# nianticlabs/relpose-gnn

Measured on AMD Instinct MI355X. Metric: graphs/sec (8-node fully-connected, 224x224), higher is better.
Workload: dtype f32; 1 GPU; BASELINE.json configs[1]: batch=32 8-node fully-connected graphs per GPU, 224x224 RGB, fp32, ResNet34 + GNN (D=2048, gnn_recursion=2, droprate=0, eval), random-init weights; nodes_per_graph=8, edges_per_graph=56, streams_per_gpu=2, loaded_library=relpose-gnn_amd/lib/librelpose_gnn_hip.so@b255fe2efddb

## Files before the change

relpose-gnn_amd/csrc/gemm_f32.hip:

```cpp
#include <atomic>
#include <map>
#include <mutex>
#include <type_traits>
#include <utility>
#include <vector>

#include "rpg_common.h"

typedef float f32x16 __attribute__((ext_vector_type(16)));

namespace {


struct Epilogue {
    const float* scale;
    const float* shift;
    const float* residual;
    float* out;
    int ldc;
    int relu;
    const int64_t* res_idx = nullptr;
    const float* residual2 = nullptr;
    const int64_t* res2_idx = nullptr;
    int ldr = 0;
// ... 520 lines not shown
    const long span = 256 / ((long)ho * wo) + 2;
    int seg = span * h * wd * cin * 4 >= (1L << 31) ? 0 : (cin % 32 == 0 ? 32 : (cin % 16 == 0 ? 16 : 0));
    if (cin == 4 && kh * kw <= 64 && kw >= 4 && span * h * wd * cin * 4 < (1L << 31)) seg = -1;
    launch_tiles<ConvKind, ConvArgs>(a, w, (int)K, (int)M, cout, (int)K, ep, s, seg);
    timing_end(slot, 2.0 * (double)M * cout * (double)kh * kw * (alg_cin > 0 ? alg_cin : cin), s, t_executed);
    RPG_CHECK_LAUNCH("conv2d_bn_act");
    return RPG_OK;
}

int launch_linear(const GatherSrc& src, const float* weight, const float* bias, const float* residual, float* out,
                  int m, int n_out, int relu, hipStream_t s, const GatherRes* gres, float* out_relu) {
    if (src.n < 1 || src.n > 3 || !weight || !out || m <= 0 || n_out <= 0 || !aligned16(weight)) return RPG_ERR_BAD_ARG;
    GatherArgs a{};
    int K = 0;
    for (int i = 0; i < 3; ++i) {
        if (i < src.n) {
            if (!src.a[i] || src.width[i] <= 0 || (src.width[i] & 3) || (src.ld[i] & 3) || src.ld[i] < src.width[i] ||
                !aligned16(src.a[i]))
                return RPG_ERR_BAD_ARG;
            a.a[i] = src.a[i]; a.idx[i] = src.idx[i]; a.ld[i] = src.ld[i];
            K += src.width[i];
        } else {
            a.a[i] = nullptr; a.idx[i] = nullptr; a.ld[i] = 0;
        }
    }
    a.w0 = src.width[0];
    a.w01 = src.n >= 2 ? src.width[0] + src.width[1] : K;
    a.K = K;
    a.fold_k = g_fold_k;
    Epilogue ep{nullptr, bias, residual, out, n_out, relu};
    ep.out_relu = out_relu;
    if (out_relu && !aligned16(out_relu)) return RPG_ERR_BAD_ARG;
    if (gres) {
        if (!gres->res1 || !gres->idx1 || gres->ld < n_out || (gres->res2 && !gres->idx2)) return RPG_ERR_BAD_ARG;
        ep.residual = gres->res1; ep.res_idx = gres->idx1;
        ep.residual2 = gres->res2; ep.res2_idx = gres->idx2;
        ep.ldr = gres->ld;
    }
    const int slot = timing_begin(RPG_TIMER_LINEAR, s);
    int seg = 32;
    for (int i = 0; i < src.n; ++i) {
        if (src.width[i] % 32) seg = src.width[i] % 16 ? 0 : (seg ? 16 : 0);
        const long rows = src.idx[i] ? src.rows[i] : (long)m;
        if (rows <= 0 || rows * src.ld[i] * 4 >= (1L << 31)) seg = 0;
    }
    if (!(src.n == 1 && !src.idx[0] && launch_linear112(src.a[0], src.ld[0], weight, K, m, n_out, K, ep, s)))
        launch_tiles<GatherKind, GatherArgs>(a, weight, K, m, n_out, K, ep, s, seg);
    timing_end(slot, 2.0 * (double)m * n_out * (double)K, s, t_executed);
    RPG_CHECK_LAUNCH("linear_gather");
    return RPG_OK;
}

}

extern "C" int rpg_conv2d_bn_act_nhwc_f32(const float* x, const float* w_ohwi, const float* scale, const float* shift,
                                          const float* residual, float* y, int n, int h, int w, int cin, int cout,
                                          int kh, int kw, int stride, int pad, int relu, void* stream) {
    return rpg::launch_conv(x, w_ohwi, scale, shift, residual, y, n, h, w, cin, cout, kh, kw, stride, pad, relu,
                            rpg::as_stream(stream));
}

extern "C" int rpg_linear_gather_f32(int n_src, const float* const* a, const int64_t* const* idx, const int* ld,
                                     const int* width, const float* weight, const float* bias, const float* residual,
                                     float* out, int m, int n_out, int relu, void* stream) {
    if (n_src < 1 || n_src > 3 || !a || !ld || !width) return RPG_ERR_BAD_ARG;
    rpg::GatherSrc src{};
    src.n = n_src;
    for (int i = 0; i < n_src; ++i) {
        src.a[i] = a[i];
        src.idx[i] = idx ? idx[i] : nullptr;
        src.ld[i] = ld[i];
        src.width[i] = width[i];
    }
    return rpg::launch_linear(src, weight, bias, residual, out, m, n_out, relu, rpg::as_stream(stream));
}

extern "C" int rpg_linear_gather_ex_f32(int n_src, const float* const* a, const int64_t* const* idx, const int* ld,
                                        const int* width, const long* rows, const float* weight, const float* bias,
                                        const float* residual, const int64_t* res_idx, const float* residual2,
                                        const int64_t* res2_idx, int ldr, float* out, float* out_relu, int m, int n_out,
                                        int relu, void* stream) {
    if (n_src < 1 || n_src > 3 || !a || !ld || !width) return RPG_ERR_BAD_ARG;
    rpg::GatherSrc src{};
    src.n = n_src;
    for (int i = 0; i < n_src; ++i) {
        src.a[i] = a[i];
        src.idx[i] = idx ? idx[i] : nullptr;
        src.ld[i] = ld[i];
        src.width[i] = width[i];
        src.rows[i] = rows ? rows[i] : 0;
    }
    if (!res_idx && !residual2)
        return (res2_idx || (residual && ldr && ldr != n_out)) ? RPG_ERR_BAD_ARG
               : rpg::launch_linear(src, weight, bias, residual, out, m, n_out, relu, rpg::as_stream(stream), nullptr, out_relu);
    rpg::GatherRes gr{residual, res_idx, residual2, res2_idx, ldr};
    return rpg::launch_linear(src, weight, bias, nullptr, out, m, n_out, relu, rpg::as_stream(stream), &gr, out_relu);
}

extern "C" int rpg_release_scratch(void) {
    if (hipDeviceSynchronize() != hipSuccess) {
        rpg::set_last_error("release_scratch", hipGetLastError());
        return RPG_ERR_LAUNCH;
    }
    std::lock_guard<std::mutex> lk(g_scratch_mu);
    for (auto& kv : g_scratch)
        if (kv.second.p) (void)hipFree(kv.second.p);
    g_scratch.clear();
    for (float* p : g_retired) (void)hipFree(p);
    g_retired.clear();
    return RPG_OK;
}

extern "C" int rpg_set_tuning(int key, int value) {
    switch (key) {
        case RPG_TUNE_FIXUP_PRIO: g_fixup_prio = value != 0; return RPG_OK;
        case RPG_TUNE_BF16_PAIR: rpg::bf16_set_pair(value != 0); return RPG_OK;
        case RPG_TUNE_TILE: g_force_tile = value; return RPG_OK;
        case RPG_TUNE_BK: if (value != 0 && value != 16 && value != 32) return RPG_ERR_BAD_ARG; g_bk = value; return RPG_OK;
        case RPG_TUNE_EPILOGUE: g_epi_lds = value != 0; return RPG_OK;
        case RPG_TUNE_STREAMK: g_streamk = value != 0; return RPG_OK;
        case RPG_TUNE_BF16_BK: if (value != 32 && value != 64) return RPG_ERR_BAD_ARG; rpg::bf16_set_bk(value); return RPG_OK;
        case RPG_TUNE_INKERNEL_FIXUP:
            if (value < 0 || value > 7) return RPG_ERR_BAD_ARG;
            g_inkernel_fixup = value & 3;
            rpg::wino_combine_max_set((value & 4) ? 32 : 8);
            return RPG_OK;
        case RPG_TUNE_GNN_SPLIT: g_gnn_split = value != 0; return RPG_OK;
        case RPG_TUNE_GNN_FUSE_AGG: g_gnn_fuse_agg = value != 0; return RPG_OK;
        case RPG_TUNE_LIN112: if (value < 0 || value > 3) return RPG_ERR_BAD_ARG; g_lin112 = value; return RPG_OK;
        case RPG_TUNE_FOLD_K: if (value < 0 || (value % 64)) return RPG_ERR_BAD_ARG; g_fold_k = value; return RPG_OK;
        case RPG_TUNE_FAST_LOADER: g_fast = value != 0; return RPG_OK;
        case RPG_TUNE_WAVES8: g_waves8 = value != 0; return RPG_OK;
        case RPG_TUNE_WINO_SPLIT: if (value < 0 || value > 96) return RPG_ERR_BAD_ARG; rpg::wino_split_set(value); return RPG_OK;
        case RPG_TUNE_BF16_TILE: if (value < -1 || value > 3) return RPG_ERR_BAD_ARG; rpg::bf16_set_tile(value); return RPG_OK;
        case RPG_TUNE_BF16_FAST: rpg::bf16_set_fast(value != 0); return RPG_OK;
        case RPG_TUNE_BF16_LEAN_EPI: rpg::bf16_set_lean_epi(value != 0); return RPG_OK;
        case RPG_TUNE_BF16_PERSIST: rpg::bf16_set_persist(value != 0); return RPG_OK;
        case RPG_TUNE_BF16_FUSE_BLOCK: rpg::bf16_set_fuse_block((int)(value & 7)); return RPG_OK;
        case RPG_TUNE_BF16_TAIL: if (value < 0 || value > 7) return RPG_ERR_BAD_ARG; rpg::bf16_set_tail(value); return RPG_OK;
        case RPG_TUNE_BF16_LINEAR_DMA: if (value != 0 && (value < 10 || value > 19)) return RPG_ERR_BAD_ARG; rpg::bf16_set_linear_dma(value); return RPG_OK;
        case RPG_TUNE_WINO2D:
            if (value < 0 || value > 2 || (value != 0 && rpg_wino43_weights_floats(1, 1) != 42)) return RPG_ERR_BAD_ARG;
            rpg::wino2d_set(value);
            return RPG_OK;
        case RPG_TUNE_BF16_CHUNK:
            if (value < 0) return RPG_ERR_BAD_ARG;
            rpg::bf16_set_chunk(value & 4095, (value >> 12) ? (value >> 12) : 64);
            return RPG_OK;
        case RPG_TUNE_BF16_PATCH: if (value < 0 || value % 10 > 4 || value > 14) return RPG_ERR_BAD_ARG; rpg::bf16_set_patch(value); return RPG_OK;
        case RPG_TUNE_BF16_DMA: if (value < 0 || value > 40) return RPG_ERR_BAD_ARG; rpg::bf16_set_dma(value); return RPG_OK;
        case RPG_TUNE_SK_MIN_ITS: if (value < 1 || value > 4096) return RPG_ERR_BAD_ARG; SK_MIN_ITS = value; return RPG_OK;
        case RPG_TUNE_BF16_WS64: if (value < 0 || value > 2) return RPG_ERR_BAD_ARG; return rpg::bf16_set_ws64(value);
        case RPG_TUNE_FUSED_STEM: rpg::stem_pool_set((value & 1) != 0); rpg::stem_pool_set_strip((value & 128) != 0, value >> 8); rpg::bf16_set_fused_stem((value & 1) != 0); rpg::bf16_set_stem_strip((value & 2) ? 0 : ((value & 32) ? 1 : 9), value >> 8); return RPG_OK;
        case RPG_TUNE_WINOGRAD: if (value < 0 || (value > 3 && value < 16)) return RPG_ERR_BAD_ARG; rpg::wino_set(value); return RPG_OK;
        case RPG_TUNE_WINO_PERSIST: if (value < 0 || value > 2) return RPG_ERR_BAD_ARG; rpg::wino_persist_set(value); return RPG_OK;
        case RPG_TUNE_WINO_SHORT: if (value < 0) return RPG_ERR_BAD_ARG; rpg::wino_short_set(value); return RPG_OK;
        default: return RPG_ERR_BAD_ARG;
    }
}
```

relpose-gnn_amd/csrc/winograd.hip:

```cpp
#include "rpg_common.h"

typedef float f32x16 __attribute__((ext_vector_type(16)));

namespace {

constexpr int NT = 256;
constexpr int BK = 16, LD = BK;
constexpr int P = 6;
constexpr int BMT = 64, BN = 64;
constexpr int A_FLOATS = P * BMT * LD, B_FLOATS = P * BN * LD;
constexpr int LDS_BYTES = (A_FLOATS + B_FLOATS) * (int)sizeof(float);

struct Epi {
    const float* scale;
    const float* shift;
    const float* residual;
    float* out;
    int relu;
};

__device__ __forceinline__ float4 f4zero() { return make_float4(0.f, 0.f, 0.f, 0.f); }
__device__ __forceinline__ float4 lin(float a, const float4& x, float b, const float4& y) {
    return make_float4(a * x.x + b * y.x, a * x.y + b * y.y, a * x.z + b * y.z, a * x.w + b * y.w);
}
// ... 776 lines not shown
                decode();
            }
        }
    };

    const int st_a = row * LD + 4 * (slot ^ ((row >> 2) & 3));
    const int st_b = A8_FLOATS + (3 * bhalf) * BN * LD + brow * LD + 4 * (slot ^ ((brow >> 2) & 3));
    struct Img { int a[2], b[2], sa, sb; };
    float4* lds4 = reinterpret_cast<float4*>(lds);
    auto stage_one = [&](int p, const Img& I) {
        if (p >= P) {
            lds4[I.sb + (p - P) * (BN * LD / 4)] = ub[p - P];
            return;
        }
#ifdef RPG_ABL_NOXF
        lds4[I.sa + p * (BMT8 * LD / 4)] = d[p];
        return;
#endif
        const F4 d0 = to_f4(d[0]), d1 = to_f4(d[1]), d2 = to_f4(d[2]), d3 = to_f4(d[3]), d4 = to_f4(d[4]), d5 = to_f4(d[5]);
        F4 v;
        if (p == 0) v = fma4_p4(sub4(d0, d2), sub4(d4, d2));
        else if (p == 5) v = fma4_m4(sub4(d3, d1), sub4(d5, d3));
        else if (p <= 2) {
            const F4 sx = fma4_m4(d2, d4);
            const F4 tx = fma4_m4(d1, d3);
            v = p == 1 ? add4(sx, tx) : sub4(sx, tx);
        } else {
            const F4 r = sub4(d4, d2), t = sub4(d3, d1);
            v = p == 3 ? fma4_p2(t, r) : fma4_m2(t, r);
        }
        lds4[I.sa + p * (BMT8 * LD / 4)] = to_float4(v);
    };

    f32x16 acc[P];
    const int rsw = 4 * ((lane >> 5) ^ ((lane >> 2) & 3));
    const int a_off = (wm * 32 + (lane & 31)) * LD + rsw;
    const int b_off = A8_FLOATS + (wn * 32 + (lane & 31)) * LD + rsw;
    float4 fa[2][2], fb[2][2];
    constexpr int IMG4 = IMG8_FLOATS / 4;
    Img X{{a_off >> 2, (a_off ^ 8) >> 2}, {b_off >> 2, (b_off ^ 8) >> 2}, st_a >> 2, st_b >> 2};
    Img Y{{X.a[0] + IMG4, X.a[1] + IMG4}, {X.b[0] + IMG4, X.b[1] + IMG4}, X.sa + IMG4, X.sb + IMG4};
    int ybase = IMG8_FLOATS;
    auto frag_one = [&](int g, int set, int i, const Img& I) {
        const int xi = 2 * (g % 3) + (i >> 1);
        if (i & 1) fb[set][i >> 1] = lds4[I.b[g / 3] + xi * (BN * LD / 4)];
        else       fa[set][i >> 1] = lds4[I.a[g / 3] + xi * (BMT8 * LD / 4)];
    };
    auto kstep = [&](const Img& cur, const Img& nxt, int khf) {
        __builtin_amdgcn_sched_barrier(0);
#pragma unroll
        for (int g = 0; g < 6; ++g) {
            const int set = g & 1, x0 = 2 * (g % 3);
#pragma unroll
            for (int i = 0; i < 8; ++i) {
                const int j = i & 1, e = i >> 1;
                const float av = e == 0 ? fa[set][j].x : e == 1 ? fa[set][j].y : e == 2 ? fa[set][j].z : fa[set][j].w;
                const float bv = e == 0 ? fb[set][j].x : e == 1 ? fb[set][j].y : e == 2 ? fb[set][j].z : fb[set][j].w;
                acc[x0 + j] = __builtin_amdgcn_mfma_f32_32x32x2f32(av, bv, acc[x0 + j], 0, 0, 0);
                if (i < 4) {
                    if (g < 5) frag_one(g + 1, set ^ 1, i, cur);
                    else frag_one(0, 0, i, nxt);
                } else {
                    const int s = 4 * (g % 3) + (i - 4);
                    if (s < 9) {
                        if (g < 3) stage_one(s, nxt);
                        else fetch_one(s, khf);
                    }
                }
                __builtin_amdgcn_sched_barrier(0);
            }
#ifndef RPG_ABL_NOBAR
            if (g == 4) {
                __syncthreads();
                __builtin_amdgcn_sched_barrier(0);
            }
#endif
        }
        fetch_next(khf);
    };

    int c_item = f_item, c_m0 = f_m0, c_n0 = f_n0, c_ns = f_nk - f_kb;
#pragma unroll
    for (int i = 0; i < 9; ++i) fetch_one(i, 0);
    fetch_next(0);
#pragma unroll
    for (int p = 0; p < 9; ++p) stage_one(p, X);
#pragma unroll
    for (int i = 0; i < 9; ++i) fetch_one(i, 1);
    fetch_next(1);
    const int ws = __builtin_amdgcn_readfirstlane(wave);
    for (;;) {
#ifdef RPG_WINO_TRACE
        if (g_wino_trace && threadIdx.x == 0) {
            g_wino_trace[5 * c_item] = __builtin_amdgcn_s_getreg(0xF804);
            g_wino_trace[5 * c_item + 1] = __builtin_readcyclecounter();
        }
#endif
#pragma unroll
        for (int xi = 0; xi < P; ++xi)
#pragma unroll
            for (int e = 0; e < 16; ++e) acc[xi][e] = 0.f;
        __syncthreads();
#pragma unroll
        for (int i = 0; i < 4; ++i) frag_one(0, 0, i, X);
#ifdef RPG_WINO_TRACE
        if (g_wino_trace && threadIdx.x == 0) g_wino_trace[5 * c_item + 2] = __builtin_readcyclecounter();
#endif
        int s = 0;
        for (; s + 6 <= c_ns; s += 6) {
            kstep(X, Y, 2);
            kstep(Y, X, 0);
            kstep(X, Y, 1);
            kstep(Y, X, 2);
            kstep(X, Y, 0);
            kstep(Y, X, 1);
        }
        if (s < c_ns) {
            kstep(X, Y, 2);
            kstep(Y, X, 0);
            kstep(X, Y, 1);
            const Img t = X;
            X = Y;
            Y = t;
            ybase = IMG8_FLOATS - ybase;
        }
        __syncthreads();
        float* slab = lds + ybase + ws * (64 * 36);
#ifdef RPG_WINO_TRACE
        if (g_wino_trace && threadIdx.x == 0) g_wino_trace[5 * c_item + 3] = __builtin_readcyclecounter();
#endif
        auto refetch = [&]() {
            fix_row1();
#pragma unroll
            for (int i = 0; i < 9; ++i) fetch_one(i, 1);
        };
        int lane_e = lane;
        asm volatile("" : "+v"(lane_e));
        if (c_item < sp.n_split)
            wino43_epilogue_partial(acc, slab, lane_e, (ws >> 1) * 32, (ws & 1) * 32,
                                    sp.partial + (size_t)c_item * (BMT8 * 4 * BN), refetch);
        else
            wino43_epilogue_lean(acc, slab, lane_e, c_m0 + (ws >> 1) * 32, c_n0 + (ws & 1) * 32, M, Tw, W, Cout, ep, refetch);
#ifdef RPG_WINO_TRACE
        if (g_wino_trace && threadIdx.x == 0) g_wino_trace[5 * c_item + 4] = __builtin_readcyclecounter();
#endif
        if (f_item >= n_items) break;
        c_item = f_item;
        c_m0 = f_m0;
        c_n0 = f_n0;
        c_ns = f_nk - f_kb;
    }
}

__global__ __launch_bounds__(256) void wino43_fixup_kernel(const float* __restrict__ partial, Epi ep, int M, int Tw, int W,
                                                           int Cout, int tiles_n, Split sp) {
    const int tt = blockIdx.x >> 5, idx = (blockIdx.x & 31) * 256 + threadIdx.x;
    const float* src = partial + (size_t)tt * sp.parts * (BMT8 * 4 * BN) + 4 * idx;
    float4 s = *reinterpret_cast<const float4*>(src);
    for (int i = 1; i < sp.parts; ++i) {
        const float4 v = *reinterpret_cast<const float4*>(src + (size_t)i * (BMT8 * 4 * BN));
        s.x += v.x; s.y += v.y; s.z += v.z; s.w += v.w;
    }
    wino43_finish_quad(s, ep, sp.tile_base + tt, idx >> 4, idx & 15, M, Tw, W, Cout, tiles_n);
}

__global__ __launch_bounds__(NT) void wino43_weights_kernel(const float* __restrict__ w, float* __restrict__ U, int Cout,
                                                            int Cin, long total) {
    const long i = (long)blockIdx.x * NT + threadIdx.x;
    if (i >= total) return;
    const int c = (int)(i % Cin);
    const long t = i / Cin;
    const int kh = (int)(t % 3);
    const long co = t / 3;
    const float* wp = w + ((co * 3 + kh) * 3) * (long)Cin + c;
    const double g0 = wp[0], g1 = wp[Cin], g2 = wp[2 * (long)Cin];
    const double u[6] = {g0 / 4.0, -(g0 + g1 + g2) / 6.0, -(g0 - g1 + g2) / 6.0,
                         g0 / 24.0 + g1 / 12.0 + g2 / 6.0, g0 / 24.0 - g1 / 12.0 + g2 / 6.0, g2};
    const long plane = (long)Cout * 3 * Cin;
#pragma unroll
    for (int xi = 0; xi < 6; ++xi) U[xi * plane + i] = (float)u[xi];
}

int g_wino_split = 1;
int g_wino_split_steps = 3;
int g_wino = 1;
int g_wino_min_blocks = 16;
int g_wino_persist = 1;
int g_wino_combine_max = 8;

}

#ifdef RPG_PROBE_WINO2D
#include "../../tools/probes/winograd2d.hip"
#endif

namespace rpg {

#ifndef RPG_PROBE_WINO2D
void wino2d_set(int) {}
#endif
bool wino_enabled() { return g_wino != 0; }
void wino_set(int on) { if (on >= 16) { g_wino = 1; g_wino_min_blocks = on; } else { g_wino = on; g_wino_min_blocks = 16; } }
void wino_split_set(int v) { g_wino_split = v != 0; g_wino_split_steps = v >= 2 ? v : 3; }
void wino_short_set(int) {}
void wino_persist_set(int on) { g_wino_persist = on; }
void wino_combine_max_set(int v) { g_wino_combine_max = v; }

bool wino_pays(int n, int h, int w, int cin, int cout) {
    if (!g_wino || (cin & 3) || (cout & 3)) return false;
    const long tiles = (long)n * h * ((w + 3) / 4);
    const long blocks = ((tiles + BMT - 1) / BMT) * ((cout + BN - 1) / BN);
    const int tw = (w + 3) / 4;
    return blocks >= g_wino_min_blocks && (long)h * w * cin * 4 * 67 < (1L << 31) && 6L * cout * 3 * cin * 4 < (1L << 31) &&
           (32L / tw + 3) * w * cout * 4 < (1L << 31);
}

int launch_conv_wino(const float* x, const float* u, const float* scale, const float* shift, const float* residual,
                     float* y, int n, int h, int w, int cin, int cout, int relu, hipStream_t s) {
    if (!x || !u || !y || n <= 0 || h <= 0 || w <= 0 || cin <= 0 || cout <= 0 || (cin & 3) || (cout & 3) ||
        !aligned16(x) || !aligned16(u) || !aligned16(y) || (scale && !aligned16(scale)) || (shift && !aligned16(shift)) ||
        (residual && !aligned16(residual)))
        return RPG_ERR_BAD_ARG;
#ifdef RPG_PROBE_WINO2D
    if (wino2d_takes(n, h, w, cin, cout))
        return launch_conv_wino2d(x, u + (size_t)18 * cout * cin, scale, shift, residual, y, n, h, w, cin, cout, relu, s);
#endif
    const int tw = (w + 3) / 4;
    const long M = (long)n * h * tw;
    if (M >= (1L << 31) || (long)h * w * cin * 4 * 67 >= (1L << 31) || 6L * cout * 3 * cin * 4 >= (1L << 31) ||
        (32L / tw + 3) * w * cout * 4 >= (1L << 31))
        return RPG_ERR_BAD_ARG;
    int dev = 0;
    if (hipGetDevice(&dev) != hipSuccess || dev < 0 || dev >= 64) dev = 0;
    static bool attr[64] = {};
    if (!attr[dev]) {
        (void)hipFuncSetAttribute(reinterpret_cast<const void*>(wino43_conv_kernel),
                                  hipFuncAttributeMaxDynamicSharedMemorySize, LDS_BYTES);
        attr[dev] = true;
    }
    const int tn = (cout + BN - 1) / BN;
    Epi ep{scale, shift, residual, y, relu};
    const int slot = timing_begin(RPG_TIMER_CONV_WINO, s);
    double executed = 0.0;
    const long tm8 = (M + BMT8 - 1) / BMT8;
    const bool fits8 = (long)h * w * cin * 4 * 131 < (1L << 31);
    if (fits8 && (g_wino == 3 || (g_wino == 1 && tm8 * tn >= 8))) {
        static bool attr8[64] = {};
        if (!attr8[dev]) {
            (void)hipFuncSetAttribute(reinterpret_cast<const void*>(wino43_conv8_kernel),
                                      hipFuncAttributeMaxDynamicSharedMemorySize, LDS8_BYTES);
            attr8[dev] = true;
        }
        const long T = tm8 * tn;
        const int S = num_cus(), kpr = (cin + BK - 1) / BK, nk = 3 * kpr;
        executed = (double)T * nk * 48.0 * 8.0 * 4096.0;
        long t_main = T;
        Split sp{0, 1, 0, nullptr, nullptr};
        const long tail = T % S;
        if (g_wino_persist && cin % BK == 0 && (T > S || g_wino_persist == 2) && h >= 2) {
            static bool attr8p[64] = {};
            if (!attr8p[dev]) {
                (void)hipFuncSetAttribute(reinterpret_cast<const void*>(wino43_conv8p_kernel),
                                          hipFuncAttributeMaxDynamicSharedMemorySize, LDS8_BYTES);
                attr8p[dev] = true;
            }
            if (g_wino_split && tail > 0) {
                int parts = (int)(S / tail);
                if (parts > kpr) parts = kpr;
                if (parts >= 2) {
                    sp.partial = stream_scratch(s, (size_t)tail * parts * (BMT8 * 4 * BN) * sizeof(float));
                    if (sp.partial) { sp.parts = parts; t_main = T - tail; sp.tile_base = (int)t_main; sp.n_split = (int)(tail * parts); }
                }
            }
            const long items = sp.n_split + t_main;
            hipLaunchKernelGGL(wino43_conv8p_kernel, dim3((unsigned)(items < S ? items : S)), dim3(NT8), LDS8_BYTES, s, x, u, h, w,
                               cin, cout, tw, (int)M, ep, tn, sp, (int)items);
            if (sp.n_split) {
                hipStream_t fs = fixup_hop_begin(s);
                hipLaunchKernelGGL(wino43_fixup_kernel, dim3((unsigned)(T - t_main) * 32), dim3(256), 0, fs, sp.partial, ep, (int)M,
                                   tw, w, cout, tn, sp);
                fixup_hop_end(s, fs);
            }
            timing_end(slot, 2.0 * (double)n * h * w * cout * 9.0 * cin, s, executed);
            RPG_CHECK_LAUNCH("conv3x3_wino43");
            return RPG_OK;
        }
        if (g_wino_split && tail > 0) {
            int parts = (int)(S / tail);
            if (parts > kpr) parts = kpr;
            if (parts > nk / g_wino_split_steps && nk / g_wino_split_steps >= 2) parts = nk / g_wino_split_steps;
            if (parts >= 2) {
                unsigned* counters = nullptr;
                sp.partial = stream_scratch(s, (size_t)tail * parts * (BMT8 * 4 * BN) * sizeof(float), &counters);
                if (sp.partial) { sp.parts = parts; t_main = T - tail; sp.tile_base = (int)t_main; sp.n_split = (int)(tail * parts); }
                if (sp.partial && inkernel_fixup_enabled() && parts <= g_wino_combine_max) sp.arrive = counters;
            }
        }
        hipLaunchKernelGGL(wino43_conv8_kernel, dim3((unsigned)(sp.n_split + t_main)), dim3(NT8), LDS8_BYTES, s, x, u, h, w, cin,
                           cout, tw, (int)M, ep, tn, sp);
        if (sp.n_split && !sp.arrive) {
            hipStream_t fs = fixup_hop_begin(s);
            hipLaunchKernelGGL(wino43_fixup_kernel, dim3((unsigned)(T - t_main) * 32), dim3(256), 0, fs, sp.partial, ep, (int)M, tw, w,
                               cout, tn, sp);
            fixup_hop_end(s, fs);
        }
    } else {
        const int tm = (int)((M + BMT - 1) / BMT);
        executed = (double)tm * tn * (3 * ((cin + BK - 1) / BK)) * 48.0 * 4.0 * 4096.0;
        hipLaunchKernelGGL(wino43_conv_kernel, dim3(tm * tn), dim3(NT), LDS_BYTES, s, x, u, h, w, cin, cout, tw, (int)M, ep, tn);
    }
    timing_end(slot, 2.0 * (double)n * h * w * cout * 9.0 * cin, s, executed);
    RPG_CHECK_LAUNCH("conv3x3_wino43");
    return RPG_OK;
}

}

#ifdef RPG_WINO_TRACE
extern "C" int rpg_wino_trace_set(unsigned long long* buf) {
    return hipMemcpyToSymbol(HIP_SYMBOL(g_wino_trace), &buf, sizeof(buf)) == hipSuccess ? RPG_OK : RPG_ERR_LAUNCH;
}
#endif

extern "C" size_t rpg_wino43_weights_floats(int cout, int cin) {
    if (cout <= 0 || cin <= 0) return 0;
#ifdef RPG_PROBE_WINO2D
    return rpg::wino_weight_floats(cout, cin);
#else
    return (size_t)18 * cout * cin;
#endif
}

extern "C" int rpg_wino43_transform_weights_f32(const float* w_ohwi, float* u, int cout, int cin, void* stream) {
    if (!w_ohwi || !u || cout <= 0 || cin <= 0) return RPG_ERR_BAD_ARG;
    const long total = (long)cout * 3 * cin;
    hipLaunchKernelGGL(wino43_weights_kernel, dim3((unsigned)((total + NT - 1) / NT)), dim3(NT), 0, rpg::as_stream(stream),
                       w_ohwi, u, cout, cin, total);
    RPG_CHECK_LAUNCH("wino43_transform_weights");
#ifdef RPG_PROBE_WINO2D
    return rpg::launch_wino2d_weights(w_ohwi, u + (size_t)18 * cout * cin, cout, cin, rpg::as_stream(stream));
#else
    return RPG_OK;
#endif
}

extern "C" int rpg_conv3x3_wino43_bn_act_nhwc_f32(const float* x, const float* u, const float* scale, const float* shift,
                                                  const float* residual, float* y, int n, int h, int w, int cin, int cout,
                                                  int relu, void* stream) {
    return rpg::launch_conv_wino(x, u, scale, shift, residual, y, n, h, w, cin, cout, relu, rpg::as_stream(stream));
}
```

Measured before the change: 3089 graphs/s.

## Add shared-row Winograd conv kernel reusing input rows across the three kernel rows

Adds a new Winograd F(4,3) conv kernel that stages one transformed input strip plus halo rows in LDS. The kh=0,1,2 kernel-row passes then read shifted windows of the same strip instead of refetching and retransforming input per kernel row. It is enabled by default when the tile width fits, for both the persistent and one-shot launch paths, with a new tune value to disable it. The kernel uses more LDS per block, which may lower occupancy, and adds complex index and halo logic.

```diff
diff --git a/relpose-gnn_amd/csrc/gemm_f32.hip b/relpose-gnn_amd/csrc/gemm_f32.hip
--- a/relpose-gnn_amd/csrc/gemm_f32.hip
+++ b/relpose-gnn_amd/csrc/gemm_f32.hip
@@ -696,7 +696,7 @@
         case RPG_TUNE_SK_MIN_ITS: if (value < 1 || value > 4096) return RPG_ERR_BAD_ARG; SK_MIN_ITS = value; return RPG_OK;
         case RPG_TUNE_BF16_WS64: if (value < 0 || value > 2) return RPG_ERR_BAD_ARG; return rpg::bf16_set_ws64(value);
         case RPG_TUNE_FUSED_STEM: rpg::stem_pool_set((value & 1) != 0); rpg::stem_pool_set_strip((value & 128) != 0, value >> 8); rpg::bf16_set_fused_stem((value & 1) != 0); rpg::bf16_set_stem_strip((value & 2) ? 0 : ((value & 32) ? 1 : 9), value >> 8); return RPG_OK;
-        case RPG_TUNE_WINOGRAD: if (value < 0 || (value > 3 && value < 16)) return RPG_ERR_BAD_ARG; rpg::wino_set(value); return RPG_OK;
+        case RPG_TUNE_WINOGRAD: if (value < 0 || (value > 4 && value < 16)) return RPG_ERR_BAD_ARG; rpg::wino_set(value); return RPG_OK;
         case RPG_TUNE_WINO_PERSIST: if (value < 0 || value > 2) return RPG_ERR_BAD_ARG; rpg::wino_persist_set(value); return RPG_OK;
         case RPG_TUNE_WINO_SHORT: if (value < 0) return RPG_ERR_BAD_ARG; rpg::wino_short_set(value); return RPG_OK;
         default: return RPG_ERR_BAD_ARG;
diff --git a/relpose-gnn_amd/csrc/winograd.hip b/relpose-gnn_amd/csrc/winograd.hip
--- a/relpose-gnn_amd/csrc/winograd.hip
+++ b/relpose-gnn_amd/csrc/winograd.hip
@@ -952,6 +952,343 @@
     }
 }
 
+constexpr int SROWS = 148, SZROW = SROWS - 4;
+constexpr int WINO_SHARED_MAX_TW = (SZROW - BMT8) / 2;
+constexpr int SPLANE = SROWS * LD, SA_FLOATS = P * SPLANE;
+constexpr int S_A0 = 0, S_B0 = SA_FLOATS, S_B1 = S_B0 + B_FLOATS, S_A1 = S_B1 + B_FLOATS;
+constexpr int LDS8S_BYTES = (2 * SA_FLOATS + 2 * B_FLOATS) * (int)sizeof(float);
+static_assert(SA_FLOATS + B_FLOATS >= 8 * 64 * 36, "the epilogue slabs fit in one (A, B) pair");
+static_assert(S_A1 % LD == 0 && S_B0 % LD == 0, "image bases keep the chunk swizzle");
+
+template <bool ONE>
+__global__ __launch_bounds__(NT8) void wino43_conv8s_kernel(const float* __restrict__ x, const float* __restrict__ U, int H,
+                                                           int W, int Cin, int Cout, int Tw, int M, Epi ep, int tiles_n,
+                                                           Split sp, int n_items) {
+    extern __shared__ __attribute__((aligned(16))) float lds[];
+    const int K = 3 * Cin;
+    const int kpr = Cin / BK;
+    const int tid = threadIdx.x, lane = tid & 63, wave = tid >> 6;
+    const int wn = wave & 1;
+    const int row = tid >> 2, slot = tid & 3;
+    const int brow = row & 63, bhalf = tid >> 8;
+    const size_t img_floats = (size_t)H * W * Cin;
+    const __amdgpu_buffer_rsrc_t rb = __builtin_amdgcn_make_buffer_rsrc(const_cast<float*>(U), 0, 0x7fffffff, 0x00020000);
+    constexpr unsigned OOB = 0x80000000u;
+    const unsigned ustride_b = (unsigned)Cout * K * 4u;
+    const unsigned krow_b = 4u * (unsigned)Cin;
+    const bool halo_lane = row < 2 * Tw;
+
+    const float rcp_tw = 1.0f / (float)Tw, rcp_h = 1.0f / (float)H;
+    struct Pos { int dn, ho, tw; };
+    auto locate = [&](int rem0, int h0, int e) -> Pos {
+        const int a = rem0 + e + Tw;
+        const int q = (int)(((float)a + 0.5f) * rcp_tw);
+        const int b = h0 + q - 1 + H;
+        const int qn = (int)(((float)b + 0.5f) * rcp_h);
+        return Pos{qn - 1, b - qn * H, a - q * Tw};
+    };
+    auto item_tile = [&](int item, int& kb, int& nk) -> int {
+        kb = 0;
+        nk = 3 * kpr;
+        if (item < sp.n_split) {
+            const int tt = item / sp.parts, part = item - tt * sp.parts;
+            kb = 3 * (part * kpr / sp.parts);
+            nk = 3 * ((part + 1) * kpr / sp.parts);
+            return sp.tile_base + tt;
+        }
+        const int nwg = n_items - sp.n_split, bid = item - sp.n_split;
+        const int xcd = bid & 7, loc = bid >> 3, q = nwg >> 3, r8 = nwg & 7;
+        return (xcd < r8 ? xcd * (q + 1) : r8 * (q + 1) + (xcd - r8) * q) + loc;
+    };
+
+    int f_item = blockIdx.x, f_m0 = 0, f_n0 = 0, f_kb = 0, f_nk = 0, f_kt = 0, f_c0 = 0;
+    unsigned vb_eff;
+    auto decode_b = [&]() {
+        asm volatile("" ::: "memory");
+        int tid_d = tid;
+        asm volatile("" : "+v"(tid_d));
+        const int slot = tid_d & 3, brow = (tid_d >> 2) & 63, bhalf = tid_d >> 8;
+        const bool valid = f_item < n_items;
+        int kb, nk;
+        const int tile = item_tile(f_item, kb, nk);
+        f_m0 = (tile / tiles_n) * BMT8;
+        f_n0 = (tile - (tile / tiles_n) * tiles_n) * BN;
+        vb_eff = valid && f_n0 + brow < Cout ? 4u * (unsigned)((f_n0 + brow) * K + 4 * slot) + 3u * bhalf * ustride_b : OOB;
+        f_kb = kb;
+        f_kt = kb;
+        f_nk = valid ? nk : 0x3fffffff;
+        f_c0 = (kb / 3) * BK;
+    };
+    int a_item = blockIdx.x, a_c0 = 0, a_cend = 0;
+    const float* a_base = x;
+    unsigned va_m[P], va_h[P];
+    auto decode_a = [&]() {
+        asm volatile("" ::: "memory");
+        int tid_d = tid;
+        asm volatile("" : "+v"(tid_d));
+        const int row = tid_d >> 2, slot = tid_d & 3;
+        const bool valid = a_item < n_items;
+        int kb, nk;
+        const int tile = item_tile(a_item, kb, nk);
+        const int m0 = (tile / tiles_n) * BMT8;
+        const int t0 = m0 / Tw, rem0 = m0 - t0 * Tw, n_first = t0 / H, h0 = t0 - n_first * H;
+        a_base = x + n_first * img_floats;
+        auto offsets = [&](int e, bool ok, int need, unsigned (&va)[P]) {
+            const Pos p = locate(rem0, h0, e);
+            const int m = m0 + e;
+            int img_off = 0, ho = 0, wi0 = -(1 << 24);
+            if (ok && m >= 0 && m < M && !(need == 1 && p.ho == H - 1) && !(need == 2 && p.ho == 0)) {
+                ho = p.ho;
+                img_off = p.dn * (int)img_floats;
+                wi0 = 4 * p.tw - 1;
+            }
+#pragma unroll
+            for (int j = 0; j < P; ++j) {
+                const int wi = wi0 + j;
+                va[j] = (unsigned)wi < (unsigned)W ? 4u * (unsigned)(img_off + (ho * W + wi) * Cin + 4 * slot) : OOB;
+            }
+        };
+        offsets(row, valid, 0, va_m);
+        const bool front = row < Tw;
+        offsets(front ? row - Tw : BMT8 + (row - Tw), valid && row < 2 * Tw, front ? 1 : 2, va_h);
+        a_c0 = (kb / 3) * BK;
+        a_cend = valid ? (nk / 3) * BK : 0x3fffffff;
+    };
+    auto advance_a = [&]() {
+        a_c0 += BK;
+        if (a_c0 >= a_cend) {
+            a_item += gridDim.x;
+            decode_a();
+        }
+    };
+    decode_b();
+    decode_a();
+
+    float4 d[P], ub[3];
+    auto fetch_a = [&](int i, bool halo) {
+        const __amdgpu_buffer_rsrc_t ra = __builtin_amdgcn_make_buffer_rsrc(const_cast<float*>(a_base), 0, 0x7fffffff, 0x00020000);
+        const unsigned sa = 4u * (unsigned)a_c0;
+        if (halo) {
+            if (halo_lane) d[i] = __builtin_bit_cast(float4, __builtin_amdgcn_raw_buffer_load_b128(ra, va_h[i], sa, 0));
+        } else
+            d[i] = __builtin_bit_cast(float4, __builtin_amdgcn_raw_buffer_load_b128(ra, va_m[i], sa, 0));
+    };
+    auto fetch_b = [&](int i, int kh) {
+        const unsigned sb = (unsigned)kh * krow_b + 4u * (unsigned)f_c0 + (unsigned)i * ustride_b;
+        ub[i] = __builtin_bit_cast(float4, __builtin_amdgcn_raw_buffer_load_b128(rb, vb_eff, sb, 0));
+    };
+    auto fetch_next = [&](int kh) {
+        ++f_kt;
+        if (kh == 2) {
+            f_c0 += BK;
+            if (f_kt >= f_nk) {
+                f_item += gridDim.x;
+                decode_b();
+            }
+        }
+    };
+
+    struct ImgS { int a[3][2], b[2], sam, sah, sb; };
+    float4* lds4 = reinterpret_cast<float4*>(lds);
+    auto swz = [](int r, int c) { return r * LD + 4 * (c ^ ((r >> 2) & 3)); };
+    ImgS X, Y;
+    if (tid < 2 * P * 16)
+        lds4[(((tid >= P * 16 ? S_A1 : S_A0) + ((tid >> 4) % P) * SPLANE + SZROW * LD) >> 2) + (tid & 15)] = f4zero();
+    int ypair = 1;
+    auto set_imgs = [&](int m0) {
+        int tid_r = tid;
+        asm volatile("" : "+v"(tid_r));
+        const int lane_r = tid_r & 63, row = tid_r >> 2, slot = tid_r & 3, brow = row & 63, bhalf = tid_r >> 8;
+        const int wv = __builtin_amdgcn_readfirstlane(tid_r >> 6);
+        const int xa = ypair ? S_A0 : S_A1, ya = ypair ? S_A1 : S_A0, xb = ypair ? S_B0 : S_B1, yb = ypair ? S_B1 : S_B0;
+        const int rm = Tw + row, rh = row < Tw ? row : BMT8 + row;
+        const int bo = ((wv & 1) * 32 + (lane_r & 31)) * LD + 4 * ((lane_r >> 5) ^ ((lane_r >> 2) & 3));
+        const int so = (3 * bhalf) * BN * LD + swz(brow, slot);
+        X.sam = (xa + swz(rm, slot)) >> 2;
+        Y.sam = (ya + swz(rm, slot)) >> 2;
+        X.sah = (xa + swz(rh, slot)) >> 2;
+        Y.sah = (ya + swz(rh, slot)) >> 2;
+        X.sb = (xb + so) >> 2;
+        Y.sb = (yb + so) >> 2;
+        X.b[0] = (xb + bo) >> 2;
+        X.b[1] = (xb + (bo ^ 8)) >> 2;
+        Y.b[0] = (yb + bo) >> 2;
+        Y.b[1] = (yb + (bo ^ 8)) >> 2;
+        const int tr = (wv >> 1) * 32 + (lane_r & 31);
+        const int t0 = m0 / Tw, rem0 = m0 - t0 * Tw, h0 = t0 - (t0 / H) * H;
+        const int ho = locate(rem0, h0, tr).ho;
+        const bool in = m0 + tr < M;
+        const bool live[3] = {in && ho > 0, in, in && ho < H - 1};
+#pragma unroll
+        for (int kh = 0; kh < 3; ++kh) {
+            const int r = kh * Tw + tr;
+            const int rz = SZROW + ((r - SZROW) & 3);
+            const int o = (live[kh] ? r : rz) * LD + 4 * ((lane_r >> 5) ^ ((r >> 2) & 3));
+            X.a[kh][0] = (xa + o) >> 2;
+            X.a[kh][1] = (xa + (o ^ 8)) >> 2;
+            Y.a[kh][0] = (ya + o) >> 2;
+            Y.a[kh][1] = (ya + (o ^ 8)) >> 2;
+        }
+    };
+    set_imgs(f_m0);
+
+    F4 x_r, x_t, x_s, x_q;
+    auto xf_piece = [&](int q) -> F4 {
+        const F4 d0 = to_f4(d[0]), d1 = to_f4(d[1]), d2 = to_f4(d[2]), d3 = to_f4(d[3]), d4 = to_f4(d[4]), d5 = to_f4(d[5]);
+        switch (q) {
+            case 0: x_r = sub4(d4, d2); return fma4_p4(sub4(d0, d2), x_r);
+            case 1: x_t = sub4(d3, d1); return fma4_p2(x_t, x_r);
+            case 2: return fma4_m2(x_t, x_r);
+            case 3: return fma4_m4(x_t, sub4(d5, d3));
+            case 4: x_s = fma4_m4(d2, d4); x_q = fma4_m4(d1, d3); return add4(x_s, x_q);
+            default: return sub4(x_s, x_q);
+        }
+    };
+    auto stage_a = [&](int q, int dst, bool halo) {
+        const int pos = q == 0 ? 0 : q <= 3 ? q + 2 : q - 3;
+        if (halo) {
+            if (halo_lane) lds4[dst + pos * (SPLANE / 4)] = to_float4(xf_piece(q));
+        } else
+            lds4[dst + pos * (SPLANE / 4)] = to_float4(xf_piece(q));
+    };
+    auto stage_b = [&](int i, const ImgS& I) { lds4[I.sb + i * (BN * LD / 4)] = ub[i]; };
+
+    f32x16 acc[P];
+    float4 fa[2][2], fb[2][2];
+    auto frag_one = [&](int g, int set, int i, const ImgS& IA, const ImgS& IB, int kh) {
+        const int xi = 2 * (g % 3) + (i >> 1);
+        if (i & 1) fb[set][i >> 1] = lds4[IB.b[g / 3] + xi * (BN * LD / 4)];
+        else       fa[set][i >> 1] = lds4[IA.a[kh][g / 3] + xi * (SPLANE / 4)];
+    };
+    auto kstep = [&](const ImgS& IA, const ImgS& IAn, const ImgS& IB, const ImgS& IBn, int kh) {
+        const int khf = (kh + 2) % 3;
+        __builtin_amdgcn_sched_barrier(0);
+#pragma unroll
+        for (int g = 0; g < 6; ++g) {
+            const int set = g & 1, x0 = 2 * (g % 3);
+#pragma unroll
+            for (int i = 0; i < 8; ++i) {
+                const int j = i & 1, e = i >> 1;
+                const float av = e == 0 ? fa[set][j].x : e == 1 ? fa[set][j].y : e == 2 ? fa[set][j].z : fa[set][j].w;
+                const float bv = e == 0 ? fb[set][j].x : e == 1 ? fb[set][j].y : e == 2 ? fb[set][j].z : fb[set][j].w;
+                acc[x0 + j] = __builtin_amdgcn_mfma_f32_32x32x2f32(av, bv, acc[x0 + j], 0, 0, 0);
+                if (i < 4) {
+                    if (g < 5) frag_one(g + 1, set ^ 1, i, IA, IB, kh);
+                    else frag_one(0, 0, i, kh == 2 ? IAn : IA, IBn, (kh + 1) % 3);
+                } else {
+                    const int s = 4 * (g % 3) + (i - 4);
+                    if (g < 3) {
+                        if (s < P) {
+                            if (kh == 1) stage_a(s, IAn.sah, true);
+                            else if (kh == 2) stage_a(s, IAn.sam, false);
+                        } else if (s < 9) stage_b(s - P, IBn);
+                    } else {
+                        if (s < P) {
+                            if (kh == 0) fetch_a(s, true);
+                            else if (kh == 1) fetch_a(s, false);
+                        } else if (s < 9) fetch_b(s - P, khf);
+                    }
+                }
+                __builtin_amdgcn_sched_barrier(0);
+            }
+            if (g == 4) {
+                __syncthreads();
+                __builtin_amdgcn_sched_barrier(0);
+            }
+        }
+        fetch_next(khf);
+        if (kh == 1) advance_a();
+    };
+
+    int c_item = f_item, c_m0 = f_m0, c_n0 = f_n0, c_ns = f_nk - f_kb;
+    {
+        float4 dh[P];
+#pragma unroll
+        for (int i = 0; i < P; ++i) fetch_a(i, false);
+#pragma unroll
+        for (int i = 0; i < P; ++i) {
+            const __amdgpu_buffer_rsrc_t ra = __builtin_amdgcn_make_buffer_rsrc(const_cast<float*>(a_base), 0, 0x7fffffff, 0x00020000);
+            dh[i] = __builtin_bit_cast(float4, __builtin_amdgcn_raw_buffer_load_b128(ra, va_h[i], 4u * (unsigned)a_c0, 0));
+        }
+#pragma unroll
+        for (int i = 0; i < 3; ++i) fetch_b(i, 0);
+        fetch_next(0);
+        advance_a();
+#pragma unroll
+        for (int q = 0; q < P; ++q) stage_a(q, X.sam, false);
+#pragma unroll
+        for (int i = 0; i < P; ++i) d[i] = dh[i];
+#pragma unroll
+        for (int q = 0; q < P; ++q) stage_a(q, X.sah, true);
+#pragma unroll
+        for (int i = 0; i < 3; ++i) stage_b(i, X);
+#pragma unroll
+        for (int i = 0; i < 3; ++i) fetch_b(i, 1);
+        fetch_next(1);
+    }
+    const int ws = __builtin_amdgcn_readfirstlane(wave);
+    for (;;) {
+#pragma unroll
+        for (int xi = 0; xi < P; ++xi)
+#pragma unroll
+            for (int e = 0; e < 16; ++e) acc[xi][e] = 0.f;
+        set_imgs(c_m0);
+        __syncthreads();
+#pragma unroll
+        for (int i = 0; i < 4; ++i) frag_one(0, 0, i, X, X, 0);
+        int s = 0;
+        for (; s + 6 <= c_ns; s += 6) {
+            kstep(X, Y, X, Y, 0);
+            kstep(X, Y, Y, X, 1);
+            kstep(X, Y, X, Y, 2);
+            kstep(Y, X, Y, X, 0);
+            kstep(Y, X, X, Y, 1);
+            kstep(Y, X, Y, X, 2);
+        }
+        if (s < c_ns) {
+            kstep(X, Y, X, Y, 0);
+            kstep(X, Y, Y, X, 1);
+            kstep(X, Y, X, Y, 2);
+            ypair ^= 1;
+        }
+        __syncthreads();
+        float* slab = lds + (ypair ? S_B1 : S_A0) + ws * (64 * 36);
+        if (ONE) {
+            if (c_item < sp.n_split) {
+                wino43_epilogue_partial(acc, slab, lane, (ws >> 1) * 32, (ws & 1) * 32, sp.partial + (size_t)c_item * (BMT8 * 4 * BN));
+                if (sp.arrive)
+                    wino43_combine_last(sp, c_item / sp.parts, ep, M, Tw, W, Cout, tiles_n,
+                                        reinterpret_cast<int*>(lds + (ypair ? S_B1 : S_A0)));
+            } else
+                wino43_epilogue(acc, slab, lane, c_m0 + (ws >> 1) * 32, c_n0 + (ws & 1) * 32, M, Tw, W, Cout, ep);
+            return;
+        }
+        auto refetch = [&]() {
+#pragma unroll
+            for (int i = 0; i < 3; ++i) fetch_b(i, 1);
+        };
+        int lane_e = lane;
+        asm volatile("" : "+v"(lane_e));
+        if (c_item < sp.n_split)
+            wino43_epilogue_partial(acc, slab, lane_e, (ws >> 1) * 32, (ws & 1) * 32,
+                                    sp.partial + (size_t)c_item * (BMT8 * 4 * BN), refetch);
+        else
+            wino43_epilogue_lean(acc, slab, lane_e, c_m0 + (ws >> 1) * 32, c_n0 + (ws & 1) * 32, M, Tw, W, Cout, ep, refetch);
+        if (f_item >= n_items) break;
+        __syncthreads();
+        int tid_z = tid;
+        asm volatile("" : "+v"(tid_z));
+        float z = 0.f;
+        asm volatile("" : "+v"(z));
+        if (tid_z < P * 16)
+            lds4[(((ypair ? S_A1 : S_A0) + (tid_z >> 4) * SPLANE + SZROW * LD) >> 2) + (tid_z & 15)] = make_float4(z, z, z, z);
+        c_item = f_item;
+        c_m0 = f_m0;
+        c_n0 = f_n0;
+        c_ns = f_nk - f_kb;
+    }
+}
+
 __global__ __launch_bounds__(256) void wino43_fixup_kernel(const float* __restrict__ partial, Epi ep, int M, int Tw, int W,
                                                            int Cout, int tiles_n, Split sp) {
     const int tt = blockIdx.x >> 5, idx = (blockIdx.x & 31) * 256 + threadIdx.x;
@@ -984,6 +1321,7 @@
 int g_wino_split = 1;
 int g_wino_split_steps = 3;
 int g_wino = 1;
+int g_wino_shared = 1;
 int g_wino_min_blocks = 16;
 int g_wino_persist = 1;
 int g_wino_combine_max = 8;
@@ -1000,7 +1338,10 @@
 void wino2d_set(int) {}
 #endif
 bool wino_enabled() { return g_wino != 0; }
-void wino_set(int on) { if (on >= 16) { g_wino = 1; g_wino_min_blocks = on; } else { g_wino = on; g_wino_min_blocks = 16; } }
+void wino_set(int on) {
+    g_wino_shared = on != 4;
+    if (on >= 16) { g_wino = 1; g_wino_min_blocks = on; } else { g_wino = on == 4 ? 3 : on; g_wino_min_blocks = 16; }
+}
 void wino_split_set(int v) { g_wino_split = v != 0; g_wino_split_steps = v >= 2 ? v : 3; }
 void wino_short_set(int) {}
 void wino_persist_set(int on) { g_wino_persist = on; }
@@ -1057,6 +1398,17 @@
         long t_main = T;
         Split sp{0, 1, 0, nullptr, nullptr};
         const long tail = T % S;
+        const bool shared = g_wino_shared && cin % BK == 0 && tw <= WINO_SHARED_MAX_TW;
+        if (shared) {
+            static bool attr8s[64] = {};
+            if (!attr8s[dev]) {
+                (void)hipFuncSetAttribute(reinterpret_cast<const void*>(wino43_conv8s_kernel<false>),
+                                          hipFuncAttributeMaxDynamicSharedMemorySize, LDS8S_BYTES);
+                (void)hipFuncSetAttribute(reinterpret_cast<const void*>(wino43_conv8s_kernel<true>),
+                                          hipFuncAttributeMaxDynamicSharedMemorySize, LDS8S_BYTES);
+                attr8s[dev] = true;
+            }
+        }
         if (g_wino_persist && cin % BK == 0 && (T > S || g_wino_persist == 2) && h >= 2) {
             static bool attr8p[64] = {};
             if (!attr8p[dev]) {
@@ -1073,8 +1425,12 @@
                 }
             }
             const long items = sp.n_split + t_main;
-            hipLaunchKernelGGL(wino43_conv8p_kernel, dim3((unsigned)(items < S ? items : S)), dim3(NT8), LDS8_BYTES, s, x, u, h, w,
-                               cin, cout, tw, (int)M, ep, tn, sp, (int)items);
+            if (shared)
+                hipLaunchKernelGGL(wino43_conv8s_kernel<false>, dim3((unsigned)(items < S ? items : S)), dim3(NT8), LDS8S_BYTES, s, x,
+                                   u, h, w, cin, cout, tw, (int)M, ep, tn, sp, (int)items);
+            else
+                hipLaunchKernelGGL(wino43_conv8p_kernel, dim3((unsigned)(items < S ? items : S)), dim3(NT8), LDS8_BYTES, s, x, u, h, w,
+                                   cin, cout, tw, (int)M, ep, tn, sp, (int)items);
             if (sp.n_split) {
                 hipStream_t fs = fixup_hop_begin(s);
                 hipLaunchKernelGGL(wino43_fixup_kernel, dim3((unsigned)(T - t_main) * 32), dim3(256), 0, fs, sp.partial, ep, (int)M,
@@ -1096,8 +1452,12 @@
                 if (sp.partial && inkernel_fixup_enabled() && parts <= g_wino_combine_max) sp.arrive = counters;
             }
         }
-        hipLaunchKernelGGL(wino43_conv8_kernel, dim3((unsigned)(sp.n_split + t_main)), dim3(NT8), LDS8_BYTES, s, x, u, h, w, cin,
-                           cout, tw, (int)M, ep, tn, sp);
+        if (shared)
+            hipLaunchKernelGGL(wino43_conv8s_kernel<true>, dim3((unsigned)(sp.n_split + t_main)), dim3(NT8), LDS8S_BYTES, s, x, u, h, w,
+                               cin, cout, tw, (int)M, ep, tn, sp, (int)(sp.n_split + t_main));
+        else
+            hipLaunchKernelGGL(wino43_conv8_kernel, dim3((unsigned)(sp.n_split + t_main)), dim3(NT8), LDS8_BYTES, s, x, u, h, w, cin,
+                               cout, tw, (int)M, ep, tn, sp);
         if (sp.n_split && !sp.arrive) {
             hipStream_t fs = fixup_hop_begin(s);
             hipLaunchKernelGGL(wino43_fixup_kernel, dim3((unsigned)(T - t_main) * 32), dim3(256), 0, fs, sp.partial, ep, (int)M, tw, w,
```

New measurement: 3106 graphs/s, median of 6. No clear change (+0.6%).
